# nils-werner/pymf

Measured on AMD Instinct MI355X. Metric: factorize_iters_per_sec, higher is better.
Workload: dtype f32

## Files before the change

### pymf_amd/csrc/pmf_fused.h

```cpp
#pragma once
#include "pmf_dev.h"
#include <hip/hip_ext.h>
#include "../../include/pymf_hip.h"
#include "pmf_fused_api.h"

#define PMF_GLDS16(gsrc, ldst)                                                            \
  __builtin_amdgcn_global_load_lds((const __attribute__((address_space(1))) void*)(gsrc), \
                                   (__attribute__((address_space(3))) void*)(ldst), 16, 0, 0)

#ifdef PMF_STAMPS
#define PMF_STAMP(var)                                                           \
  do {                                                                           \
    __builtin_amdgcn_sched_barrier(0);                                           \
    asm volatile("s_memtime %0\n\ts_waitcnt lgkmcnt(0)" : "=s"(var)::"memory"); \
    __builtin_amdgcn_sched_barrier(0);                                           \
  } while (0)
#else
#define PMF_STAMP(var) do { } while (0)
#endif


__device__ __forceinline__ void slab_store16(f32x4* p, f32x4 v) { *p = v; }
__device__ __forceinline__ void wrow_store(float* p, float v) { *p = v; }

template <int N>
__device__ __forceinline__ void wait_vmcnt() {
  static_assert(N >= 0 && N < 64, "vmcnt range");
  asm volatile("s_waitcnt vmcnt(%0)" ::"n"(N) : "memory");
}

template <int NT, int NPANEL, int SPLIT = 1>
constexpr size_t fused_smem_bytes() {
  return (size_t)64 * (SPLIT * NPANEL * 16 * NT + 16 * NT + 4 * 16 * NPANEL + 4 * 16) * sizeof(float) +
         (SPLIT == 2 ? (size_t)4 * NT * 1024 : 0);
}

__device__ __forceinline__ int vtile_xor(int row) { return (row ^ ((row & 4) << 1)) & 15; }
__device__ __forceinline__ int vtile_off(int row, int chunk) { return row * 64 + ((chunk ^ vtile_xor(row)) << 2); }
__device__ __forceinline__ f32x4 vtile_read4(const float* base, int row, int chunk) {
  return *reinterpret_cast<const f32x4*>(base + vtile_off(row, chunk));
}

template <int NT, int NPANEL, int MODE, int SPLIT = 1>
__global__ __launch_bounds__(256, 1) void k_nmf_fused(const float* __restrict__ V,
                                                       float* __restrict__ W,
                                                       const float* __restrict__ H,
                                                       const float* __restrict__ G, int blk_per,
                                                       int blk_extra, float lamb,
                                                       float* __restrict__ slab,
                                                       const FusedCtl ctl, int ngp
#ifdef PMF_STAMPS
                                                       , unsigned long long* __restrict__ dbg
#endif
                                                       ) {
  constexpr int KP = 16 * NT;
  static_assert(SPLIT == 1 || (SPLIT == 2 && MODE != FUSED_SNMF), "SPLIT: 1, or 2 for the NMF/BNMF epilogues");
  constexpr int NPT = NPANEL * SPLIT;
  constexpr int NP = 64 * NPT;
  constexpr int NTP = 4 * NPANEL;
  constexpr bool SPREAD = (NPANEL == 4);
  constexpr bool SNMF = (MODE == FUSED_SNMF);
  if (ctl.stop != nullptr && *ctl.stop != 0) return;
#ifdef PMF_STAMPS
  unsigned long long tk0 = 0, tk1 = 0, tk2 = 0, tk3 = 0;
  const unsigned long long rt0 = wall_clock64();
  PMF_STAMP(tk0);
#endif
  extern __shared__ __attribute__((aligned(16))) float smem[];
  float* sH = smem;
  float* sG = sH + NPT * KP * 64;
  float* sVall = sG + KP * 64;
  float* sWall = sVall + 4 * NPANEL * 16 * 64;
  const int tid = threadIdx.x, lane = tid & 63;
  const int wv = __builtin_amdgcn_readfirstlane(tid >> 6);
  const int i = lane & 15, kq = lane >> 4;
  float* sV = sVall + wv * (NPANEL * 1024);
  float* sW = sWall + wv * 1024;
  f32x4* sX = reinterpret_cast<f32x4*>(sWall + 4 * 1024);
  const int half = SPLIT == 2 ? (wv & 1) : 0;
  const int hp = half * NPANEL;

  const int gw = SPLIT == 2 ? blockIdx.x * 2 + (wv >> 1) : blockIdx.x * 4 + wv;
  const int b0 = gw * blk_per + (gw < blk_extra ? gw : blk_extra);
  const int nb = blk_per + (gw < blk_extra ? 1 : 0);
  const int nb_wg = blk_per + (blk_extra > 0 ? 1 : 0);
  constexpr bool interleave = NT == 1;
  const int nw_all = (int)gridDim.x * (SPLIT == 2 ? 2 : 4);
  const int bfirst = interleave ? gw : b0;
  const int bstep = interleave ? nw_all : 1;

  unsigned voff[4], woff[4];
#pragma unroll
  for (int q = 0; q < 4; ++q) {
    const int row = 4 * q + (lane >> 4);
    const int c = (lane & 15) ^ vtile_xor(row);
    voff[q] = (unsigned)(row * NP * 4 + 16 * c);
    woff[q] = (unsigned)(row * KP * 4 + 16 * (4 * c < KP ? c : 0));
  }
  const char* Vb = reinterpret_cast<const char*>(V);
  const char* Wb = reinterpret_cast<const char*>(W);
  auto issue_v = [&](int blk, int p, int q) {
    PMF_GLDS16(Vb + ((size_t)blk * (16 * NP * 4) + (hp + p) * 256) + voff[q], sV + p * 1024 + q * 256);
  };
  auto issue_w = [&](int blk, int q) {
    PMF_GLDS16(Wb + (size_t)blk * (16 * KP * 4) + woff[q], sW + q * 256);
  };

  f32x4 P[NT][NTP];
  f32x4 S[NT][NT];
#pragma unroll
  for (int mt = 0; mt < NT; ++mt) {
#pragma unroll
    for (int nt = 0; nt < NTP; ++nt) P[mt][nt] = f32x4{0.f, 0.f, 0.f, 0.f};
#pragma unroll
    for (int nt = 0; nt < NT; ++nt) S[mt][nt] = f32x4{0.f, 0.f, 0.f, 0.f};
  }

  constexpr int HP = SPLIT * NT;
  constexpr int GP = SNMF ? 0 : NT;
  constexpr int WP = SNMF ? 0 : 4;
  {
    const int drow = lane >> 4, dchunk = lane & 15;
#pragma unroll
    for (int st = 0; st < NPANEL; ++st) {
#pragma unroll
      for (int hh = 0; hh < SPLIT; ++hh)
#pragma unroll
        for (int u = 0; u < NT; ++u) {
          const int p = hh * NPANEL + st, rg = 4 * u + wv;
          const int row = 4 * rg + drow;
          const int bas = NT * (row & 15) + (row >> 4);
          const float* src = H + (size_t)bas * NP + 64 * p + 4 * (dchunk ^ (row & 15));
          PMF_GLDS16(src, sH + p * (KP * 64) + rg * 256);
        }
      if (nb > 0 && (st < NPANEL - 1 || !SPREAD)) {
#pragma unroll
        for (int q = 0; q < 4; ++q) issue_v(bfirst, st, q);
      }
      if (st == 0 && !SNMF && nb > 0) {
#pragma unroll
        for (int q = 0; q < 4; ++q) issue_w(bfirst, q);
      }
    }
#pragma unroll
    for (int u = 0; u < (SNMF ? 0 : NT); ++u) {
      const int rg = 4 * u + wv;
      const int row = 4 * rg + drow;
      const int bas = NT * (row & 15) + (row >> 4);
      int c = dchunk ^ (row & 15);
      if (4 * c >= KP) c = 0;
      if (ngp == 0) {
        PMF_GLDS16(G + bas * KP + 4 * c, sG + rg * 256);
      } else {
        f32x4 g = {0.f, 0.f, 0.f, 0.f};
        for (int w = 0; w < ngp; ++w)
          g += *reinterpret_cast<const f32x4*>(G + (size_t)w * KP * KP + bas * KP + 4 * c);
        *reinterpret_cast<f32x4*>(sG + rg * 256 + drow * 64 + dchunk * 4) = g;
      }
    }
  }
  if (ctl.stop != nullptr && ctl.conv_iter >= 0) {
    double t0 = ctl.tt[0], t1 = ctl.tt[1];
    for (int q = 1; q < ctl.ntt; ++q) { t0 += ctl.tt[2 * q]; t1 += ctl.tt[2 * q + 1]; }
    const double e2 = ctl.vnorm2 - 2.0 * t0 + t1;
    int st = 0;
    if (!(e2 > 1e-3 * ctl.vnorm2)) {
      st = 2;
    } else {
      const double f = sqrt(e2);
      if (blockIdx.x == 0 && tid == 0) ctl.ferr[ctl.conv_iter] = f;
      if (ctl.conv_iter > 1 && fabs(f - ctl.ferr[ctl.conv_iter - 1]) / ctl.nsamp < ctl.eps) st = 1;
    }
    if (st != 0) {
      if (blockIdx.x == 0 && tid == 0) { ctl.stop[1] = ctl.conv_iter; ctl.stop[0] = st; }
      return;
    }
  }
  auto wg_barrier = [&]() {
    asm volatile("s_waitcnt lgkmcnt(0)" ::: "memory");
    __builtin_amdgcn_s_barrier();
    asm volatile("" ::: "memory");
  };
  auto first_stage = [&](int st) {
    if (st >= NPANEL - 1) wait_vmcnt<0>();
    else if (SPREAD) {
      if (st == 0) wait_vmcnt<WP + 2 * (HP + 4) + HP + GP>();
      else if (st == 1) wait_vmcnt<(HP + 4) + HP + GP + 3>();
      else wait_vmcnt<HP + GP + 4>();
    } else {
      if (st == 0) wait_vmcnt<WP + (NPANEL - 1) * (HP + 4) + GP>();
      else if (st == 1) wait_vmcnt<(NPANEL > 2 ? (NPANEL - 2) * (HP + 4) : 0) + GP>();
      else if (st == 2) wait_vmcnt<(NPANEL > 3 ? (NPANEL - 3) * (HP + 4) : 0) + GP>();
      else if (st == 3) wait_vmcnt<(NPANEL > 4 ? (NPANEL - 4) * (HP + 4) : 0) + GP>();
      else wait_vmcnt<0>();
    }
    wg_barrier();
  };
  if (nb == 0) {
    wait_vmcnt<0>();
#pragma unroll
    for (int st = 0; st < NPANEL; ++st) wg_barrier();
  }

  f32x4 fa[2];
  f32x4 fb[2][NT];
  f32x4 bf[2];
  f32x4 wp[NT];
#pragma unroll
  for (int nt = 0; nt < NT; ++nt) wp[nt] = f32x4{0.f, 0.f, 0.f, 0.f};

  constexpr int NSN = 4 * NPANEL;
  constexpr int NSA = SNMF ? NSN : NSN + NT;

#ifdef PMF_STAMPS
  PMF_STAMP(tk1);
  unsigned long long ts0 = 0, ts1 = 0, ts2 = 0, ts3 = 0, ts4 = 0, ts5 = 0;
  unsigned long long acc_wait = 0, acc_a = 0, acc_dma = 0, acc_epi = 0, acc_b = 0;
#endif
  for (int b = 0; b < (SPLIT == 2 ? nb_wg : nb); ++b) {
    if (SPLIT == 2) {
      wg_barrier();
      if (b >= nb) { wg_barrier(); continue; }
    }
    const int blk = bfirst + b * bstep;
    const bool more = (b + 1 < nb);
    PMF_STAMP(ts0);

    f32x4 num[NT], den[NT];
#pragma unroll
    for (int nt = 0; nt < NT; ++nt) {
      num[nt] = f32x4{0.f, 0.f, 0.f, 0.f};
      den[nt] = f32x4{0.f, 0.f, 0.f, 0.f};
    }
    auto load_step = [&](int s, int buf) {
      if (s < NSN) {
        const int p = s >> 2, chunk = 4 * (s & 3) + kq;
        fa[buf] = vtile_read4(sV + p * 1024, i, chunk);
#pragma unroll
        for (int nt = 0; nt < NT; ++nt) fb[buf][nt] = lds_read4(sH + (hp + p) * (KP * 64), 16 * nt + i, chunk);
      } else {
        const int chunk = 4 * (s - NSN) + kq;
        fa[buf] = vtile_read4(sW, i, chunk);
#pragma unroll
        for (int nt = 0; nt < NT; ++nt) fb[buf][nt] = lds_read4(sG, 16 * nt + i, chunk);
      }
    };
    auto wait_panel = [&](int p) {
      if (SPREAD) {
        if (p == 0) wait_vmcnt<8>();
        else if (p == 1) wait_vmcnt<7>();
        else if (p == 2) wait_vmcnt<4>();
        else wait_vmcnt<0>();
      } else {
        if (p == 0) wait_vmcnt<4 * (NPANEL - 1)>();
        else if (p == 1) wait_vmcnt<(NPANEL > 1 ? 4 * (NPANEL - 2) : 0)>();
        else if (p == 2) wait_vmcnt<(NPANEL > 2 ? 4 * (NPANEL - 3) : 0)>();
        else wait_vmcnt<0>();
      }
    };

    const bool first = (b == 0);
    if (first) first_stage(0);
    else wait_panel(0);
    PMF_STAMP(ts1);
    load_step(0, 0);
#pragma unroll
    for (int s = 0; s < NSA; ++s) {
      if (s + 1 < NSA) {
        if (s + 1 < NSN && ((s + 1) & 3) == 0) {
          if (first) first_stage((s + 1) >> 2);
          else wait_panel((s + 1) >> 2);
        }
        load_step(s + 1, (s + 1) & 1);
      }
      const int buf = s & 1;
      if (s < NSN) {
#pragma unroll
        for (int e = 0; e < 4; ++e)
#pragma unroll
          for (int nt = 0; nt < NT; ++nt) num[nt] = mfma16(fa[buf][e], fb[buf][nt][e], num[nt]);
      } else {
#pragma unroll
        for (int e = 0; e < 4; ++e)
#pragma unroll
          for (int nt = 0; nt < NT; ++nt) den[nt] = mfma16(fa[buf][e], fb[buf][nt][e], den[nt]);
      }
      if (SPREAD && s < 4) issue_v(blk, NPANEL - 1, s);
      if (s + 1 < NSA) {
#pragma unroll
        for (int g = 0; g < NT + 1; ++g) {
          __builtin_amdgcn_sched_group_barrier(0x008, NT >= 4 ? 2 : 1, 0);
          __builtin_amdgcn_sched_group_barrier(0x100, 1, 0);
        }
      }
      __builtin_amdgcn_sched_group_barrier(0x008, 4 * NT, 0);
      __builtin_amdgcn_sched_barrier(0);
    }
    if (SPLIT == 2) {
#pragma unroll
      for (int nt = 0; nt < NT; ++nt) sX[(wv * NT + nt) * 64 + lane] = num[nt];
      wg_barrier();
#pragma unroll
      for (int nt = 0; nt < NT; ++nt) num[nt] += sX[((wv ^ 1) * NT + nt) * 64 + lane];
    }
    PMF_STAMP(ts2);
    float wold[NT][4];
    if (!SNMF) {
#pragma unroll
      for (int nt = 0; nt < NT; ++nt)
#pragma unroll
        for (int j = 0; j < 4; ++j) {
          const int row = 4 * kq + j, col = NT * i + nt;
          wold[nt][j] = sW[vtile_off(row, col >> 2) + (col & 3)];
        }
      asm volatile("s_waitcnt lgkmcnt(0)" ::: "memory");
      if (more) {
#pragma unroll
        for (int q = 0; q < 4; ++q) issue_w(blk + bstep, q);
      }
    }
    PMF_STAMP(ts3);

    f32x4 wn[NT];
    float* wdst = W + (size_t)blk * (16 * KP) + (4 * kq) * KP + NT * i;
    if (MODE != FUSED_SNMF) {
      float tnum[NT][4], dd[NT][4], rr[NT][4], qq[NT][4];
      constexpr int NSM = 4 * (NT * (NT + 1) / 2);
      auto s_mfmas = [&](int lo, int hi) {
        if (SPLIT == 1 || half == 0) {
          int q = 0;
#pragma unroll
          for (int j = 0; j < 4; ++j)
#pragma unroll
            for (int nt = 0; nt < NT; ++nt)
#pragma unroll
              for (int mt = 0; mt <= nt; ++mt) {
                if (q >= lo && q < hi) S[mt][nt] = mfma16(wp[mt][j], wp[nt][j], S[mt][nt]);
                ++q;
              }
        }
      };
#pragma unroll
      for (int nt = 0; nt < NT; ++nt)
#pragma unroll
        for (int j = 0; j < 4; ++j) {
          const float w0 = wold[nt][j];
          if (MODE == FUSED_BNMF) {
            tnum[nt][j] = num[nt][j] + (3.0f * lamb) * (w0 * w0);
            dd[nt][j] = ((den[nt][j] + (2.0f * lamb) * (w0 * w0 * w0)) + lamb * w0) + PMF_EPS_DEN;
          } else if (MODE == FUSED_RNMF) {
            const float x = num[nt][j];
            tnum[nt][j] = fabsf(x) - x;
            dd[nt][j] = 2.0f * den[nt][j];
          } else {
            tnum[nt][j] = w0 * num[nt][j];
            dd[nt][j] = den[nt][j] + PMF_EPS_DEN;
          }
        }
      s_mfmas(0, NSM / 5);
      __builtin_amdgcn_sched_barrier(0);
#pragma unroll
      for (int nt = 0; nt < NT; ++nt)
#pragma unroll
        for (int j = 0; j < 4; ++j) rr[nt][j] = __builtin_amdgcn_rcpf(dd[nt][j]);
      s_mfmas(NSM / 5, 2 * NSM / 5);
      __builtin_amdgcn_sched_barrier(0);
#pragma unroll
      for (int nt = 0; nt < NT; ++nt)
#pragma unroll
        for (int j = 0; j < 4; ++j) qq[nt][j] = tnum[nt][j] * rr[nt][j];
      s_mfmas(2 * NSM / 5, 3 * NSM / 5);
      __builtin_amdgcn_sched_barrier(0);
#pragma unroll
      for (int nt = 0; nt < NT; ++nt)
#pragma unroll
        for (int j = 0; j < 4; ++j) tnum[nt][j] = fmaf(-dd[nt][j], qq[nt][j], tnum[nt][j]);
      s_mfmas(3 * NSM / 5, 4 * NSM / 5);
      __builtin_amdgcn_sched_barrier(0);
#pragma unroll
      for (int nt = 0; nt < NT; ++nt)
#pragma unroll
        for (int j = 0; j < 4; ++j) {
          float w = fmaf(tnum[nt][j], rr[nt][j], qq[nt][j]);
          if (MODE == FUSED_BNMF) w = wold[nt][j] * w;
          if (MODE == FUSED_RNMF) w = dd[nt][j] != 0.f ? wold[nt][j] * w : 0.f;
          wn[nt][j] = w;
          if (SPLIT == 1 || half == 0) wrow_store(&wdst[j * KP + nt], w);
        }
      s_mfmas(4 * NSM / 5, NSM);
      __builtin_amdgcn_sched_barrier(0);
    } else {
#pragma unroll
      for (int nt = 0; nt < NT; ++nt)
#pragma unroll
        for (int j = 0; j < 4; ++j) {
          const float w = num[nt][j];
          wn[nt][j] = w;
          wrow_store(&wdst[j * KP + nt], w);
#pragma unroll
          for (int mt = 0; mt <= nt; ++mt) S[mt][nt] = mfma16(wp[mt][j], wp[nt][j], S[mt][nt]);
        }
    }
#pragma unroll
    for (int nt = 0; nt < NT; ++nt) wp[nt] = wn[nt];

    PMF_STAMP(ts4);
    auto load_bf = [&](int s, int buf) {
      const int p = s >> 2, row = 4 * kq + (s & 3);
      bf[buf] = vtile_read4(sV + p * 1024, row, i);
    };
    load_bf(0, 0);
#pragma unroll
    for (int s = 0; s < NSN; ++s) {
      if (s + 1 < NSN) load_bf(s + 1, (s + 1) & 1);
      const int p = s >> 2, j = s & 3, buf = s & 1;
#pragma unroll
      for (int mt = 0; mt < NT; ++mt)
#pragma unroll
        for (int nt = 0; nt < 4; ++nt)
          P[mt][4 * p + nt] = mfma16(wn[mt][j], bf[buf][nt], P[mt][4 * p + nt]);
      if (SPREAD) {
        if (p >= 1 && more) issue_v(blk + bstep, p - 1, j);
      }
      if (s + 1 < NSN) {
        __builtin_amdgcn_sched_group_barrier(0x008, NT >= 2 ? 2 : 1, 0);
        __builtin_amdgcn_sched_group_barrier(0x100, 1, 0);
      }
      __builtin_amdgcn_sched_barrier(0);
      if (!SPREAD && j == 3) {
        asm volatile("s_waitcnt lgkmcnt(0)" ::: "memory");
        if (more) {
#pragma unroll
          for (int q = 0; q < 4; ++q) issue_v(blk + bstep, p, q);
        }
      }
    }
    if (SPREAD) asm volatile("s_waitcnt lgkmcnt(0)" ::: "memory");
#ifdef PMF_STAMPS
    PMF_STAMP(ts5);
    acc_wait += ts1 - ts0; acc_a += ts2 - ts1; acc_dma += ts3 - ts2; acc_epi += ts4 - ts3; acc_b += ts5 - ts4;
#endif
  }
#ifdef PMF_STAMPS
  PMF_STAMP(tk2);
#endif
  if (SPLIT == 1 || half == 0) {
#pragma unroll
    for (int j = 0; j < 4; ++j)
#pragma unroll
      for (int nt = 0; nt < NT; ++nt)
#pragma unroll
        for (int mt = 0; mt <= nt; ++mt) S[mt][nt] = mfma16(wp[mt][j], wp[nt][j], S[mt][nt]);
  }

  constexpr int NTU = NT * NTP + NT * (NT + 1) / 2;
  __syncthreads();
  f32x4* ex = reinterpret_cast<f32x4*>(smem);
  static_assert((size_t)2 * NTU * 64 * 16 <= fused_smem_bytes<NT, NPANEL, SPLIT>(), "exchange fits");
  auto put = [&](int region) {
    f32x4* dst = ex + (size_t)region * NTU * 64 + lane;
#pragma unroll
    for (int mt = 0; mt < NT; ++mt) {
#pragma unroll
      for (int nt = 0; nt < NTP; ++nt) dst[(mt * NTP + nt) * 64] = P[mt][nt];
#pragma unroll
      for (int nt = mt; nt < NT; ++nt)
        dst[(NT * NTP + mt * NT - (mt * (mt - 1)) / 2 + (nt - mt)) * 64] = S[mt][nt];
    }
  };
  auto add = [&](int region) {
    const f32x4* src = ex + (size_t)region * NTU * 64 + lane;
#pragma unroll
    for (int mt = 0; mt < NT; ++mt) {
#pragma unroll
      for (int nt = 0; nt < NTP; ++nt) P[mt][nt] += src[(mt * NTP + nt) * 64];
#pragma unroll
      for (int nt = mt; nt < NT; ++nt)
        S[mt][nt] += src[(NT * NTP + mt * NT - (mt * (mt - 1)) / 2 + (nt - mt)) * 64];
    }
  };
  if (wv >= 2) put(wv - 2);
  __syncthreads();
  if (wv < 2) add(wv);
  __syncthreads();
  if (wv < 2) put(wv);
  __syncthreads();
  if (SPLIT == 1) {
    f32x4* out = reinterpret_cast<f32x4*>(slab) + (size_t)blockIdx.x * NTU * 64 + lane;
    for (int t = wv; t < NTU; t += 4)
      slab_store16(&out[t * 64], ex[t * 64 + lane] + ex[(size_t)NTU * 64 + t * 64 + lane]);
  } else {
    constexpr int NTPT = 4 * NPT, NTUT = NT * NTPT + NT * (NT + 1) / 2;
    f32x4* out = reinterpret_cast<f32x4*>(slab) + (size_t)blockIdx.x * NTUT * 64 + lane;
    for (int t = wv; t < 2 * NT * NTP; t += 4) {
      const int h = t / (NT * NTP), q = t % (NT * NTP), mt = q / NTP, nt = q % NTP;
      slab_store16(&out[(mt * NTPT + h * NTP + nt) * 64], ex[(size_t)h * NTU * 64 + q * 64 + lane]);
    }
    for (int t = wv; t < NT * (NT + 1) / 2; t += 4)
      slab_store16(&out[(NT * NTPT + t) * 64], ex[(NT * NTP + t) * 64 + lane]);
  }
#ifdef PMF_STAMPS
  PMF_STAMP(tk3);
  if (dbg && lane == 0) {
    unsigned long long* d = dbg + ((size_t)blockIdx.x * 4 + wv) * 12;
    d[0] = acc_wait; d[1] = acc_a; d[2] = acc_dma; d[3] = acc_epi; d[4] = acc_b; d[5] = (unsigned long long)nb;
    d[6] = tk1 - tk0; d[7] = tk3 - tk2;
    d[8] = rt0; d[9] = wall_clock64(); d[10] = tk3 - tk0; d[11] = tk2 - tk1;
  }
#endif
}

#ifndef PMF_FUSED_KERNEL_ONLY
static inline bool fused_shape_ok(int NT, int np) {
  const int npanel = np / 64;
  if (np % 64 != 0 || npanel < 1) return false;
  const int max_panels = NT == 1 ? 6 : NT == 2 ? 5 : NT == 4 ? 4 : 0;
  return npanel <= max_panels;
}

static inline bool fused_shape_split(int NT, int np) {
  if (NT == 2) return np == 384 || np == 512;
  if (NT == 1) return np == 512;
  return false;
}

static inline int fused_grid_for(int NT, int np, int64_t mp, bool allow_split = true) {
  const bool split = allow_split && !fused_shape_ok(NT, np) && fused_shape_split(NT, np);
  if (!fused_shape_ok(NT, np) && !split) return 0;
  int dev = 0, cus = 256;
  hipDeviceProp_t prop;
  if (hipGetDevice(&dev) == hipSuccess && hipGetDeviceProperties(&prop, dev) == hipSuccess)
    cus = prop.multiProcessorCount;
  const int64_t nblk = mp / 16;
  int64_t wgs = split ? (nblk + 1) / 2 : (nblk + 3) / 4;
  if (wgs > cus) wgs = cus;
  return (int)wgs;
}

static inline const char* fused_kernel_name(int NT, int np, int mode = FUSED_NMF) {
  static char buf[64];
  const bool split = !fused_shape_ok(NT, np) && fused_shape_split(NT, np) && mode != FUSED_SNMF;
  snprintf(buf, sizeof(buf), "k_nmf_fused<%d,%d%s%s>", NT, split ? np / 128 : np / 64,
           mode == FUSED_SNMF ? ",snmf" : mode == FUSED_BNMF ? ",bnmf" : mode == FUSED_RNMF ? ",rnmf" : "", split ? ",SPLIT 2" : "");
  return buf;
}

template <int NT, int NPANEL, int MODE, int SPLIT = 1>
static int launch_fused_t(hipStream_t s, const float* V, float* W, const float* H, const float* G,
                          int64_t mp, int wgs, float lamb, float* slab, const FusedCtl& ctl, int ngp,
                          hipEvent_t e0, hipEvent_t e1) {
  const int nblk = (int)(mp / 16), nw = wgs * (SPLIT == 2 ? 2 : 4);
  const int blk_per = nblk / nw, blk_extra = nblk % nw;
  const size_t smem = fused_smem_bytes<NT, NPANEL, SPLIT>();
  static bool attr_done_dev[PMF_MAX_DEVICES] = {};
  bool& attr_done = attr_done_dev[pmf_current_device()];
  if (!attr_done) {
    if (hipFuncSetAttribute(reinterpret_cast<const void*>(&k_nmf_fused<NT, NPANEL, MODE, SPLIT>),
                            hipFuncAttributeMaxDynamicSharedMemorySize, (int)smem) != hipSuccess)
      return PMF_EHIP;
    attr_done = true;
  }
  if (e0 != nullptr && e1 != nullptr)
    hipExtLaunchKernelGGL((k_nmf_fused<NT, NPANEL, MODE, SPLIT>), dim3(wgs), dim3(256), (uint32_t)smem, s, e0, e1, 0u, V, W, H, G, blk_per,
                          blk_extra, lamb, slab, ctl, ngp);
  else
    hipLaunchKernelGGL((k_nmf_fused<NT, NPANEL, MODE, SPLIT>), dim3(wgs), dim3(256), smem, s, V, W, H, G, blk_per,
                       blk_extra, lamb, slab, ctl, ngp);
  return PMF_OK;
}

static inline int launch_fused(hipStream_t s, int mode, int NT, int np, const float* V, float* W,
                               const float* H, const float* G, int64_t mp, int wgs, float lamb,
                               float* slab, const FusedCtl& ctl, int ngp = 0, hipEvent_t e0 = nullptr, hipEvent_t e1 = nullptr) {
  if (!fused_shape_ok(NT, np) && fused_shape_split(NT, np) && mode != FUSED_SNMF) {
    const int skey = NT * 10 + np / 128;
#define PMF_FUSED_SPLIT_CASE(K, A, B)                                                                   \
  case K:                                                                                               \
    return mode == FUSED_BNMF   ? launch_fused_t<A, B, FUSED_BNMF, 2>(s, V, W, H, G, mp, wgs, lamb, slab, ctl, ngp, e0, e1) \
           : mode == FUSED_RNMF ? launch_fused_t<A, B, FUSED_RNMF, 2>(s, V, W, H, G, mp, wgs, lamb, slab, ctl, ngp, e0, e1) \
                                : launch_fused_t<A, B, FUSED_NMF, 2>(s, V, W, H, G, mp, wgs, lamb, slab, ctl, ngp, e0, e1);
    switch (skey) {
      PMF_FUSED_SPLIT_CASE(14, 1, 4)
      PMF_FUSED_SPLIT_CASE(23, 2, 3)
      PMF_FUSED_SPLIT_CASE(24, 2, 4)
    }
#undef PMF_FUSED_SPLIT_CASE
    return PMF_EINVAL;
  }
  const int key = NT * 10 + np / 64;
#define PMF_FUSED_CASE(K, A, B)                                                                  \
  case K:                                                                                        \
    return mode == FUSED_SNMF   ? launch_fused_t<A, B, FUSED_SNMF>(s, V, W, H, G, mp, wgs, lamb, slab, ctl, ngp, e0, e1) \
           : mode == FUSED_BNMF ? launch_fused_t<A, B, FUSED_BNMF>(s, V, W, H, G, mp, wgs, lamb, slab, ctl, ngp, e0, e1) \
           : mode == FUSED_RNMF ? launch_fused_t<A, B, FUSED_RNMF>(s, V, W, H, G, mp, wgs, lamb, slab, ctl, ngp, e0, e1) \
                                : launch_fused_t<A, B, FUSED_NMF>(s, V, W, H, G, mp, wgs, lamb, slab, ctl, ngp, e0, e1);
  switch (key) {
    PMF_FUSED_CASE(11, 1, 1)
    PMF_FUSED_CASE(12, 1, 2)
    PMF_FUSED_CASE(13, 1, 3)
    PMF_FUSED_CASE(14, 1, 4)
    PMF_FUSED_CASE(15, 1, 5)
    PMF_FUSED_CASE(16, 1, 6)
    PMF_FUSED_CASE(21, 2, 1)
    PMF_FUSED_CASE(22, 2, 2)
    PMF_FUSED_CASE(23, 2, 3)
    PMF_FUSED_CASE(24, 2, 4)
    PMF_FUSED_CASE(25, 2, 5)
    PMF_FUSED_CASE(41, 4, 1)
    PMF_FUSED_CASE(42, 4, 2)
    PMF_FUSED_CASE(43, 4, 3)
    PMF_FUSED_CASE(44, 4, 4)
  }
#undef PMF_FUSED_CASE
  return PMF_EINVAL;
}
#endif
```

Measured before the change: 1613.

## Switch global-to-LDS loads to buffer DMA and overlap W prefetch with final MFMAs

Global-to-LDS copies now use raw buffer loads with a buffer resource and immediate offsets instead of global_load_lds, which cuts per-lane address arithmetic. The old-W LDS reads move into the second-to-last MFMA step, and the next block's W prefetch is interleaved with the last denominator MFMAs rather than issued after the loop. The first B-fragment LDS read is hoisted ahead of the W update. This shortens the serial gap between the accumulation loop and the update stage, but it adds scheduling constraints and relies on LDS reads finishing before the W buffer is overwritten.

```diff
diff --git a/pymf_amd/csrc/pmf_fused.h b/pymf_amd/csrc/pmf_fused.h
--- a/pymf_amd/csrc/pmf_fused.h
+++ b/pymf_amd/csrc/pmf_fused.h
@@ -7,6 +7,15 @@
 #define PMF_GLDS16(gsrc, ldst)                                                            \
   __builtin_amdgcn_global_load_lds((const __attribute__((address_space(1))) void*)(gsrc), \
                                    (__attribute__((address_space(3))) void*)(ldst), 16, 0, 0)
+
+typedef __attribute__((address_space(3))) void* pmf_lds_ptr;
+__device__ __forceinline__ __amdgpu_buffer_rsrc_t dma_rsrc(const char* base, int bytes) {
+  return __builtin_amdgcn_make_buffer_rsrc(const_cast<char*>(base), 0, bytes, 0x00020000);
+}
+template <int IMM>
+__device__ __forceinline__ void dma16(__amdgpu_buffer_rsrc_t r, float* ldst, unsigned voff, int soff) {
+  __builtin_amdgcn_raw_ptr_buffer_load_lds(r, (pmf_lds_ptr)ldst, 16, (int)voff, soff, IMM, 0);
+}
 
 #ifdef PMF_STAMPS
 #define PMF_STAMP(var)                                                           \
@@ -94,16 +103,22 @@
   for (int q = 0; q < 4; ++q) {
     const int row = 4 * q + (lane >> 4);
     const int c = (lane & 15) ^ vtile_xor(row);
-    voff[q] = (unsigned)(row * NP * 4 + 16 * c);
+    voff[q] = (unsigned)(row * NP * 4 + 16 * c - 1024 * q);
     woff[q] = (unsigned)(row * KP * 4 + 16 * (4 * c < KP ? c : 0));
   }
   const char* Vb = reinterpret_cast<const char*>(V);
   const char* Wb = reinterpret_cast<const char*>(W);
   auto issue_v = [&](int blk, int p, int q) {
-    PMF_GLDS16(Vb + ((size_t)blk * (16 * NP * 4) + (hp + p) * 256) + voff[q], sV + p * 1024 + q * 256);
+    const __amdgpu_buffer_rsrc_t r = dma_rsrc(Vb + (size_t)blk * (16 * NP * 4), 16 * NP * 4);
+    float* dst = sV + p * 1024;
+    const int soff = (hp + p) * 256;
+    if (q == 0) dma16<0>(r, dst, voff[0], soff);
+    else if (q == 1) dma16<1024>(r, dst, voff[1], soff);
+    else if (q == 2) dma16<2048>(r, dst, voff[2], soff);
+    else dma16<3072>(r, dst, voff[3], soff);
   };
   auto issue_w = [&](int blk, int q) {
-    PMF_GLDS16(Wb + (size_t)blk * (16 * KP * 4) + woff[q], sW + q * 256);
+    dma16<0>(dma_rsrc(Wb + (size_t)blk * (16 * KP * 4), 16 * KP * 4), sW + q * 256, woff[q], 0);
   };
 
   f32x4 P[NT][NTP];
@@ -245,6 +260,16 @@
         for (int nt = 0; nt < NT; ++nt) fb[buf][nt] = lds_read4(sG, 16 * nt + i, chunk);
       }
     };
+    float wold[NT][4];
+    auto read_wold = [&]() {
+#pragma unroll
+      for (int nt = 0; nt < NT; ++nt)
+#pragma unroll
+        for (int j = 0; j < 4; ++j) {
+          const int row = 4 * kq + j, col = NT * i + nt;
+          wold[nt][j] = sW[vtile_off(row, col >> 2) + (col & 3)];
+        }
+    };
     auto wait_panel = [&](int p) {
       if (SPREAD) {
         if (p == 0) wait_vmcnt<8>();
@@ -279,19 +304,36 @@
         for (int e = 0; e < 4; ++e)
 #pragma unroll
           for (int nt = 0; nt < NT; ++nt) num[nt] = mfma16(fa[buf][e], fb[buf][nt][e], num[nt]);
+      } else if (s < NSA - 1) {
+#pragma unroll
+        for (int e = 0; e < 4; ++e)
+#pragma unroll
+          for (int nt = 0; nt < NT; ++nt) den[nt] = mfma16(fa[buf][e], fb[buf][nt][e], den[nt]);
       } else {
-#pragma unroll
-        for (int e = 0; e < 4; ++e)
+        asm volatile("s_waitcnt lgkmcnt(0)" ::: "memory");
+#pragma unroll
+        for (int e = 0; e < 4; ++e) {
 #pragma unroll
           for (int nt = 0; nt < NT; ++nt) den[nt] = mfma16(fa[buf][e], fb[buf][nt][e], den[nt]);
+          if (more) issue_w(blk + bstep, e);
+          __builtin_amdgcn_sched_barrier(0);
+        }
       }
       if (SPREAD && s < 4) issue_v(blk, NPANEL - 1, s);
+      if (!SNMF && s == NSA - 2) read_wold();
       if (s + 1 < NSA) {
 #pragma unroll
         for (int g = 0; g < NT + 1; ++g) {
           __builtin_amdgcn_sched_group_barrier(0x008, NT >= 4 ? 2 : 1, 0);
           __builtin_amdgcn_sched_group_barrier(0x100, 1, 0);
         }
+        if (!SNMF && s == NSA - 2) {
+#pragma unroll
+          for (int g = 0; g < 4; ++g) {
+            __builtin_amdgcn_sched_group_barrier(0x008, 1, 0);
+            __builtin_amdgcn_sched_group_barrier(0x100, 1, 0);
+          }
+        }
       }
       __builtin_amdgcn_sched_group_barrier(0x008, 4 * NT, 0);
       __builtin_amdgcn_sched_barrier(0);
@@ -304,21 +346,11 @@
       for (int nt = 0; nt < NT; ++nt) num[nt] += sX[((wv ^ 1) * NT + nt) * 64 + lane];
     }
     PMF_STAMP(ts2);
-    float wold[NT][4];
-    if (!SNMF) {
-#pragma unroll
-      for (int nt = 0; nt < NT; ++nt)
-#pragma unroll
-        for (int j = 0; j < 4; ++j) {
-          const int row = 4 * kq + j, col = NT * i + nt;
-          wold[nt][j] = sW[vtile_off(row, col >> 2) + (col & 3)];
-        }
-      asm volatile("s_waitcnt lgkmcnt(0)" ::: "memory");
-      if (more) {
-#pragma unroll
-        for (int q = 0; q < 4; ++q) issue_w(blk + bstep, q);
-      }
-    }
+    auto load_bf = [&](int s, int buf) {
+      const int p = s >> 2, row = 4 * kq + (s & 3);
+      bf[buf] = vtile_read4(sV + p * 1024, row, i);
+    };
+    load_bf(0, 0);
     PMF_STAMP(ts3);
 
     f32x4 wn[NT];
@@ -405,11 +437,6 @@
     for (int nt = 0; nt < NT; ++nt) wp[nt] = wn[nt];
 
     PMF_STAMP(ts4);
-    auto load_bf = [&](int s, int buf) {
-      const int p = s >> 2, row = 4 * kq + (s & 3);
-      bf[buf] = vtile_read4(sV + p * 1024, row, i);
-    };
-    load_bf(0, 0);
 #pragma unroll
     for (int s = 0; s < NSN; ++s) {
       if (s + 1 < NSN) load_bf(s + 1, (s + 1) & 1);
```

Result: faster. 1633, median of 6 (+1.2%).
